# valkey-io/valkey-search

Measured on AMD Instinct MI355X. Metric: kNN queries/sec + recall@10, 10M×768 fp32 cosine, flat & HNSW, 1/2/4/8 GPU, higher is better.
Workload: dtype f32; 1 GPU; FLAT 10000000x768 fp32 COSINE k=10 batch=256 (BASELINE.json configs[1]); rows_per_gpu=10000000

## Files before the change

__graft_entry__.py:

```python
import sys
from pathlib import Path

ROOT = Path(__file__).resolve().parent
sys.path.insert(0, str(ROOT))


def build() -> None:
    import subprocess
    import _pkg
    _pkg.vsa.build()
    assert _pkg.vsa.LIB_PATH.exists()
    _pkg.vsa.lib()
    from oracle import oracle as O
    O.build(ref=True)
    _pkg.vsa.build_experiments()
    subprocess.check_call(["/opt/rocm/bin/hipcc", "--offload-arch=gfx950", "-O2", "-shared", "-fPIC",
                           str(ROOT / "tests" / "helpers" / "mfma_probe.hip"), "-o", str(ROOT / "tests" / "helpers" / "libmfmaprobe.so")])
    subprocess.check_call(["/opt/rocm/bin/hipcc", "--offload-arch=gfx950", "-O2", "-shared", "-fPIC", "-I", str(_pkg.vsa.LIB_PATH.parent / "csrc"),
                           str(ROOT / "tests" / "helpers" / "prefilter_probe.hip"), "-o", str(ROOT / "tests" / "helpers" / "libprefilterprobe.so")])
    subprocess.check_call(["/opt/rocm/bin/hipcc", "--offload-arch=gfx950", "-O2", "-shared", "-fPIC", "-I", str(_pkg.vsa.LIB_PATH.parent / "csrc"),
                           str(ROOT / "tests" / "helpers" / "filter_probe.hip"), "-o", str(ROOT / "tests" / "helpers" / "libfilterprobe.so")])
    subprocess.check_call(["g++", "-O2", "-std=c++17", "-fPIC", "-shared", "-I", str(ROOT / "include"), str(ROOT / "scripts" / "serving_probe.cc"),
                           "-L", str(_pkg.vsa.LIB_PATH.parent), "-lvkindex", "-lpthread",
                           "-Wl,-rpath,$ORIGIN/../" + _pkg.vsa.LIB_PATH.parent.name, "-o", str(ROOT / "scripts" / "libservingprobe.so")])
    subprocess.check_call(["g++", "-O2", "-std=c++17", "-fPIC", "-shared", "-I", str(ROOT / "include"), "-I", str(ROOT / "tests" / "helpers"),
                           str(ROOT / "scripts" / "adaptor_probe.cc"), "-L", str(_pkg.vsa.LIB_PATH.parent), "-lvkindex", "-lpthread",
                           "-Wl,-rpath,$ORIGIN/../" + _pkg.vsa.LIB_PATH.parent.name, "-o", str(ROOT / "scripts" / "libadaptorprobe.so")])
    subprocess.check_call(["g++", "-O2", "-std=c++17", "-I", str(ROOT / "include"), str(ROOT / "scripts" / "coalescer_native.cc"),
                           "-L", str(_pkg.vsa.LIB_PATH.parent), "-lvkindex", "-lpthread",
                           "-Wl,-rpath,$ORIGIN/../" + _pkg.vsa.LIB_PATH.parent.name, "-o", str(ROOT / "scripts" / "coalescer_native")])


def smoke() -> None:
    import numpy as np
    import _pkg
    from oracle import oracle as O
# ... 38 lines not shown
```

valkey-search_amd/csrc/flat_filter.hip:

```cpp
#include <stdlib.h>

#include "device_common.hpp"
#include "kernels.hpp"

namespace vk {

typedef _Float16 f16x8 __attribute__((ext_vector_type(8)));
typedef _Float16 f16x4 __attribute__((ext_vector_type(4)));
typedef float f32x16 __attribute__((ext_vector_type(16)));

#ifdef VK_EXPERIMENTS
__device__ __forceinline__ uint32_t exp_ablate(const FlatFilterArgs &a) { return a.ablate; }
__device__ __forceinline__ uint32_t exp_prio(const FlatFilterArgs &a) { return a.prio; }
__device__ __forceinline__ unsigned long long *exp_dbg(const FlatFilterArgs &a) { return a.dbg; }
#else
__device__ __forceinline__ uint32_t exp_ablate(const FlatFilterArgs &) { return 0u; }
__device__ __forceinline__ uint32_t exp_prio(const FlatFilterArgs &) { return 0u; }
__device__ __forceinline__ unsigned long long *exp_dbg(const FlatFilterArgs &) { return nullptr; }
#endif

namespace {
constexpr int kFTileRows = 128;
constexpr int kFStageK = 64;
constexpr int kFAStride = 72;
}

__global__ __launch_bounds__(256) void row_stats_kernel(const void *rows, uint32_t bf16, uint32_t l2, uint32_t stride_e, uint32_t chunks,
                                                        uint32_t lo, uint32_t hi, uint32_t *stats, uint32_t *tile_norm, uint32_t *hn16,
                                                        _Float16 *rows16) {
  const int lane = threadIdx.x & 63, wave = threadIdx.x >> 6, j = lane & 3, rq = lane >> 2;
  const uint32_t total_waves = gridDim.x * 4, n_tiles = (hi - lo + kRowsPerWave - 1) / kRowsPerWave;
  float best_n2 = 0.f, best_abs = 0.f;
  for (uint32_t tile = blockIdx.x * 4 + wave; tile < n_tiles; tile += total_waves) {
    const uint32_t row = lo + tile * kRowsPerWave + rq;
    const uint32_t lrow = row < hi ? row : hi - 1;
    float n2 = 0.f, mx = 0.f;
    bool bad = false;
    for (uint32_t c = 0; c < chunks; ++c) {
      const float4 x = bf16 ? row_piece<true>(row_base<true>(rows, lrow, stride_e), c * 4 + j)
// ... 461 lines not shown
#pragma unroll
    for (int u = 0; u < kPieces; ++u)
      tn[u] = a.tile_norm[((size_t)((uint32_t)u * a.n_tiles + tile) * kR + i0) * a.sample_gap >> 7];
#pragma unroll
    for (int u = 0; u < kPieces; ++u) pz |= (tn[u] > cap_bits ? 1u : 0u) << u;
  }
  s.pz = pz;
#pragma unroll
  for (int u = 0; u < kPieces; ++u) {
    const size_t run = (size_t)((uint32_t)u * a.n_tiles + tile) * kR * a.sample_gap;
    const u32x4v v = __builtin_amdgcn_raw_buffer_load_b128(ws_rsrc(base + run * row_bytes), (int)voff, 0, 2);
    if constexpr (kBf16) s.v[u] = v;
    else s.v[u] = __builtin_bit_cast(f32x4v, v);
  }
}
template <bool kBf16, bool kL2, bool kSample, bool kBfMma = false>
__device__ __forceinline__ void ws_rows_store(_Float16 *buf, uint32_t *hn_buf, uint32_t t, const WsRows<kBf16> &s, bool raw = false) {
  if constexpr (kL2) hn_buf[t] = s.hn;
  if constexpr (kBf16) {
    _Float16 *dst = buf + (t >> 3) * kFAStride + (t & 7) * 8;
    if (kBfMma || raw) {
#pragma unroll
      for (int u = 0; u < 8; ++u) {
        u32x4v v = s.v[u];
        if constexpr (kSample) {
          if ((t & 7) == 0 && ((s.pz >> u) & 1u)) v[0] = (v[0] & 0xFFFF0000u) | 0x7FC0u;
        }
        *reinterpret_cast<u32x4v *>(dst + u * 16 * kFAStride) = v;
      }
      return;
    }
#pragma unroll
    for (int u = 0; u < 8; ++u) {
      f16x8 h;
#pragma unroll
      for (int w = 0; w < 4; ++w) {
        h[2 * w] = (_Float16)__uint_as_float(s.v[u][w] << 16);
        h[2 * w + 1] = (_Float16)__uint_as_float(s.v[u][w] & 0xFFFF0000u);
      }
      if constexpr (kSample) {
        if ((t & 7) == 0 && ((s.pz >> u) & 1u)) h[0] = __builtin_bit_cast(_Float16, (uint16_t)0x7E00);
      }
      *reinterpret_cast<f16x8 *>(dst + u * 16 * kFAStride) = h;
    }
  } else {
    _Float16 *dst = buf + (t >> 4) * kFAStride + (t & 15) * 4;
#pragma unroll
    for (int u = 0; u < 16; ++u) {
      f16x4 h;
      h[0] = (_Float16)s.v[u][0];
      h[1] = (_Float16)s.v[u][1];
      h[2] = (_Float16)s.v[u][2];
      h[3] = (_Float16)s.v[u][3];
      if constexpr (kSample) {
        if ((t & 15) == 0 && ((s.pz >> u) & 1u)) h[0] = __builtin_bit_cast(_Float16, (uint16_t)0x7E00);
      }
      *reinterpret_cast<f16x4 *>(dst + u * 8 * kFAStride) = h;
    }
  }
}
constexpr int kWsBStage = 8 * 4 * kWave;
constexpr int kWsThreads = 512;
__device__ __forceinline__ void ws_b_load(WsB &b, const FlatFilterArgs &a, uint32_t p, uint32_t st, uint32_t lane) {
  const uint32_t ks_n = a.row_stride_f / 16;
#pragma unroll
  for (int t4 = 0; t4 < 4; ++t4) {
    const uint32_t jt0 = p * 4 + t4, jt = jt0 < a.nqt ? jt0 : a.nqt - 1;
    const __amdgpu_buffer_rsrc_t r = ws_rsrc(reinterpret_cast<const char *>(a.q16) + ((size_t)jt * ks_n + st * 4) * kWave * 16);
#pragma unroll
    for (int kk = 0; kk < 4; ++kk) b.v[t4 * 4 + kk] = __builtin_amdgcn_raw_buffer_load_b128(r, (int)(lane * 16 + kk * 1024), 0, 0);
  }
}
__device__ __forceinline__ void ws_b_store(uint4 *slot, uint32_t p, uint32_t lane, const WsB &b) {
  u32x4v *dst = reinterpret_cast<u32x4v *>(slot) + (p * 16) * kWave + lane;
#pragma unroll
  for (int i = 0; i < 16; ++i) dst[i * kWave] = b.v[i];
}

typedef __bf16 bf16x8 __attribute__((ext_vector_type(8)));
template <bool kBfMma> __device__ __forceinline__ f32x16 ws_mfma(f16x8 x, f16x8 y, f32x16 c) {
  if constexpr (kBfMma) return __builtin_amdgcn_mfma_f32_32x32x16_bf16(__builtin_bit_cast(bf16x8, x), __builtin_bit_cast(bf16x8, y), c, 0, 0, 0);
  else return __builtin_amdgcn_mfma_f32_32x32x16_f16(x, y, c, 0, 0, 0);
}
constexpr int kDmaRing = 5;
constexpr uint32_t kDmaStageBytes = kFTileRows * 128;
constexpr int kBRing = 3;
template <bool kBf16, bool kL2, bool kTiming, bool kSample, int kAbl = 0, bool kBfMma = false, bool kDma = false, bool kBDma = false>
__device__ __forceinline__ void flat_filter_body(const FlatFilterArgs &a) {
  static_assert(!kBDma || (!kDma && !kTiming && !kSample && kAbl == 0), "B by DMA: rows through registers, final pass, no experiment variants");
  static_assert(!kDma || (kBf16 && !kL2 && !kSample && !kTiming), "the DMA row path serves a 16-bit row stream in the final pass");
  const uint32_t abl = kAbl != 0 ? exp_ablate(a) : 0u;
  extern __shared__ _Float16 lds_a[];
  constexpr uint32_t kBufHalfs = kFTileRows * kFAStride;
  uint4 *lds_b = reinterpret_cast<uint4 *>(lds_a + (kDma ? kDmaRing * kDmaStageBytes / 2 : 2 * kBufHalfs));
  uint32_t *lds_ring = reinterpret_cast<uint32_t *>(lds_b + (kBDma ? kBRing : 2) * kWsBStage);
  uint32_t *hn_lds = lds_ring + 4 * kRingWords;
  volatile __attribute__((address_space(3))) uint32_t *lds_stop =
      (volatile __attribute__((address_space(3))) uint32_t *)(hn_lds + 2 * kFTileRows);
  const uint32_t tid = threadIdx.x, lane = tid & 63;
  const uint32_t wave = __builtin_amdgcn_readfirstlane(tid >> 6);
  const uint32_t stages = a.row_stride_f / kFStageK;

  const uint32_t n_tiles = a.n_tiles;
  const uint32_t t_base = n_tiles / gridDim.x, t_rem = n_tiles % gridDim.x;
  uint32_t first_tile = blockIdx.x * t_base + (blockIdx.x < t_rem ? blockIdx.x : t_rem);
  uint32_t my_tiles = t_base + (blockIdx.x < t_rem ? 1u : 0u);
  if constexpr (!kSample) {
    if (a.part_tiles != 0) {
// ... 225 lines not shown
    }
    VK_WS_ROWS_LOAD(x0)
    fpos_advance(ld, stages);
    VK_WS_ROWS_LOAD(x1)
    fpos_advance(ld, stages);
    VK_WS_ROWS_LOAD(x2)
    fpos_advance(ld, stages);
    if constexpr (kBf16) {
      VK_WS_ROWS_LOAD(x3)
      fpos_advance(ld, stages);
      VK_WS_ROWS_LOAD(x4)
      fpos_advance(ld, stages);
      VK_WS_ROWS_LOAD(x5)
      fpos_advance(ld, stages);
    }
    ws_rows_store<kBf16, kL2, kSample, kBfMma>(lds_a, hn_lds, t, x0);
    VK_WS_PBARRIER()
    uint32_t ppar = 0;
    unsigned long long ph[4] = {0, 0, 0, 0}, tlast = __builtin_readcyclecounter();
#define VK_WS_PROD(RLOAD, RSTORE)                                                                                   \
    {                                                                                                               \
      const bool live = left_c != 0;                                                                                \
      VK_WS_TICK(3)                                                                                                 \
      if (live && st_c == 0 && t == 0 && a.cancel && (tile_c % kCancelPollTiles) == 0) {                            \
        if (__hip_atomic_load(a.cancel, __ATOMIC_RELAXED, __HIP_MEMORY_SCOPE_SYSTEM) != 0) lds_stop[tile_c & 1] = 1; \
      }                                                                                                             \
      if (!(abl & 8u)) VK_WS_ROWS_LOAD(RLOAD)                                                                       \
      fpos_advance(ld, stages);                                                                                     \
      __builtin_amdgcn_sched_barrier(0);                                                                            \
      VK_WS_TICK(0)                                                                                                 \
      ppar ^= 1;                                                                                                    \
      if (!(abl & 4u)) ws_rows_store<kBf16, kL2, kSample, kBfMma>(lds_a + ppar * kBufHalfs, hn_lds + ppar * kFTileRows, t, RSTORE, (abl & 512u) != 0); \
      else if (abl & 1024u) {         \
        _Pragma("unroll") for (int u_ = 0; u_ < (kBf16 ? 8 : 16); ++u_) asm volatile("" ::"v"(RSTORE.v[u_]));       \
      }                                                                                                             \
      if constexpr (timing) asm volatile("s_waitcnt lgkmcnt(0)" ::: "memory");                                      \
      VK_WS_TICK(2)                                                                                                 \
      left_c -= live ? 1u : 0u;                                                                                     \
      st_c += 1;                                                                                                    \
      if (live && st_c == stages) VK_WS_TILE_END(VK_WS_PBARRIER()) else VK_WS_PBARRIER();                           \
    }
    while (left_c != 0 && !stop) {
      VK_WS_PROD(x0, x1)
      if (stop) break;
      VK_WS_PROD(x1, x2)
      if (stop) break;
      if constexpr (kBf16) {
// ... 31 lines not shown
    const bool have = wave * 2 + t2 < a.nqt;
    const uint32_t jc = have ? (wave * 2 + t2) * 32 + li : 0u;
    const float4 co = a.qcoef[jc];
    closed[t2] = !have || co.w != 0.f;
    if constexpr (kSample) {
      wit[t2] = a.qwit[jc] + 0x1p-21f;
      col[t2].c1 = col[t2].c0 = col[t2].bound = 0.f;
      if constexpr (kL2) col[t2].c2 = 0.f;
    } else {
      wit[t2] = 0.f;
      if constexpr (kL2) col[t2].c2 = co.x;
      col[t2].c1 = co.y;
      col[t2].c0 = co.z;
      col[t2].bound = (closed[t2] || abl != 0) ? __builtin_inff() : a.qbound[jc];
    }
  }
  f32x16 acc[2][4];
  const f32x16 zero = {0.f, 0.f, 0.f, 0.f, 0.f, 0.f, 0.f, 0.f, 0.f, 0.f, 0.f, 0.f, 0.f, 0.f, 0.f, 0.f};
#pragma unroll
  for (int t2 = 0; t2 < 2; ++t2)
#pragma unroll
    for (int rt = 0; rt < 4; ++rt) acc[t2][rt] = zero;
  uint32_t tile_row0 = first_tile * row_step;
  uint32_t par = 0;
  const __amdgpu_buffer_rsrc_t tile_rsrc = ws_rsrc(a.tile_norm);
  uint32_t norm_bits = 0;
  if constexpr (!kSample) norm_bits = __builtin_amdgcn_raw_buffer_load_b32(tile_rsrc, 0, (int)((tile_row0 / (uint32_t)kFTileRows) * 4u), 0);
  __syncthreads();

#define VK_WS_AB(FA, FB0, FB1, KK)                                                                                  \
// ... 19 lines not shown
    VK_WS_AB(fa, b0, b1, 0)                                                                                         \
    VK_WS_AB(fb, b2, b3, 1)                                                                                         \
    MM0(fa, b0, b1)                                                                                                 \
    VK_WS_AB(fa, b0, b1, 2)                                                                                         \
    VK_WS_MM(fb, b2, b3)                                                                                            \
    VK_WS_AB(fb, b2, b3, 3)                                                                                         \
    VK_WS_MM(fa, b0, b1)                                                                                            \
    VK_WS_MM(fb, b2, b3)                                                                                            \
    __builtin_amdgcn_sched_group_barrier(0x100, 12, 0);                                                             \
    __builtin_amdgcn_sched_group_barrier(0x008, 8, 0);                                                              \
    __builtin_amdgcn_sched_group_barrier(0x100, 6, 0);                                                              \
    __builtin_amdgcn_sched_group_barrier(0x008, 8, 0);                                                              \
    __builtin_amdgcn_sched_group_barrier(0x100, 6, 0);                                                              \
    __builtin_amdgcn_sched_group_barrier(0x008, 16, 0);                                                             \
  }
  f16x8 abl_a[4], abl_b[2];
  if constexpr (kAbl != 0) {
#pragma unroll
    for (int rt = 0; rt < 4; ++rt) abl_a[rt] = *reinterpret_cast<const f16x8 *>(lds_a + li * kFAStride + g * 8 + rt * 32 * kFAStride);
    abl_b[0] = reinterpret_cast<const f16x8 *>(lds_b)[lane];
    abl_b[1] = reinterpret_cast<const f16x8 *>(lds_b)[lane + kWave];
  }
  const uint32_t dma_off = li * 128u + ((g ^ ((li >> 1) & 7u)) * 16u);
  uint32_t dma_slot = 0, b_slot = 0;
  unsigned long long ph[3] = {0, 0, 0}, tlast = __builtin_readcyclecounter();
  while (left_c != 0 && !stop) {
    VK_WS_TICK(2)
    const _Float16 *ab = lds_a + par * kBufHalfs + li * kFAStride + g * 8;
    const char *dma_ab = reinterpret_cast<const char *>(lds_a) + dma_slot;
    const f16x8 *bb = reinterpret_cast<const f16x8 *>(lds_b + (kBDma ? b_slot : par * kWsBStage) + (wave * 2) * 4 * kWave) + lane;
    if (has_q) {
      if (st_c == 0) VK_WS_STAGE(VK_WS_MMZ) else VK_WS_STAGE(VK_WS_MM)
      if constexpr ((kAbl & 128) != 0) VK_WS_STAGE(VK_WS_MM)
      if constexpr (kL2) {
        if (st_c + 1 == stages) {
          const uint4 nb = make_uint4(g == 0 ? 0xBC00BC00u : 0u, 0u, 0u, 0u);
#pragma unroll
          for (int rt = 0; rt < 4; ++rt) {
            const uint4 na = make_uint4(g == 0 ? hn_lds[par * kFTileRows + rt * 32 + li] : 0u, 0u, 0u, 0u);
            acc[0][rt] = __builtin_amdgcn_mfma_f32_32x32x16_f16(__builtin_bit_cast(f16x8, na), __builtin_bit_cast(f16x8, nb), acc[0][rt], 0, 0, 0);
            acc[1][rt] = __builtin_amdgcn_mfma_f32_32x32x16_f16(__builtin_bit_cast(f16x8, na), __builtin_bit_cast(f16x8, nb), acc[1][rt], 0, 0, 0);
          }
        }
      }
    }
    if constexpr (timing) asm volatile("s_nop 7\n s_nop 7" ::: "memory");
    VK_WS_TICK(0)
    left_c -= 1;
    st_c += 1;
    par ^= 1;
    if constexpr (kDma) dma_slot = dma_slot + kDmaStageBytes == kDmaRing * kDmaStageBytes ? 0u : dma_slot + kDmaStageBytes;
    if constexpr (kBDma) b_slot = b_slot + kWsBStage == kBRing * kWsBStage ? 0u : b_slot + kWsBStage;
    if (st_c == stages) {
      if (has_q) {
        if constexpr (kSample) {
          sample_max<4, kBf16>(a, acc[0], wit[0], closed[0], tile_row0, (wave * 2) * 32 + li, g);
          sample_max<4, kBf16>(a, acc[1], wit[1], closed[1], tile_row0, (wave * 2 + 1) * 32 + li, g);
        } else if constexpr ((kAbl & 64) != 0) {
#pragma unroll
          for (int rt = 0; rt < 4; ++rt) asm volatile("" ::"v"(acc[0][rt]), "v"(acc[1][rt]));
        } else {
          filter_gate<4, false>(a, acc[0], gate_thr<kL2>(col[0], norm_bits), tile_row0, wave * 2, li, g, ring, lane);
          filter_gate<4, false>(a, acc[1], gate_thr<kL2>(col[1], norm_bits), tile_row0, wave * 2 + 1, li, g, ring, lane);
        }
      }
      tile_row0 += row_step;
      if constexpr (!kSample) norm_bits = __builtin_amdgcn_raw_buffer_load_b32(tile_rsrc, 0, (int)((tile_row0 / (uint32_t)kFTileRows) * 4u), 0);
      VK_WS_TICK(1)
      VK_WS_TILE_END(__syncthreads())
    } else {
      __syncthreads();
    }
  }
#undef VK_WS_AB
#undef VK_WS_MM
#undef VK_WS_MMZ
#undef VK_WS_STAGE
#undef VK_WS_TILE_END
#undef VK_WS_TICK
  if constexpr (timing) {
    if (lane == 0 && exp_dbg(a))
      for (int i = 0; i < 3; ++i) atomicAdd(&exp_dbg(a)[5 + i], ph[i]);
  }
  ring_flush(a, ring, lane);
}


template <bool kBf16, bool kL2, bool kTiming, int kAbl = 0>
__global__ __launch_bounds__(kWsThreads, 1) void flat_filter_kernel(FlatFilterArgs a) {
  flat_filter_body<kBf16, kL2, kTiming, false, kAbl>(a);
}
__global__ __launch_bounds__(kWsThreads, 1) void flat_filter_bfmma_kernel(FlatFilterArgs a) {
  flat_filter_body<true, false, false, false, 0, true>(a);
}
__global__ __launch_bounds__(kWsThreads, 1) void flat_filter_bfmma_dma_kernel(FlatFilterArgs a) {
  flat_filter_body<true, false, false, false, 0, true, true>(a);
}
template <bool kBf16, bool kL2, bool kBfMma, bool kImage = false>
__global__ __launch_bounds__(kWsThreads, 1) void flat_filter_bdma_kernel(FlatFilterArgs a) {
  static_assert(!kImage || (!kBf16 && !kL2 && !kBfMma), "the f16 image belongs to f32 rows in the inner-product space");
  if constexpr (kImage) flat_filter_body<true, false, false, false, 0, false, true>(a);
  else flat_filter_body<kBf16, kL2, false, false, 0, kBfMma, false, true>(a);
}
template <bool kBf16, bool kL2, bool kBfMma, bool kImage = false>
__global__ __launch_bounds__(kWsThreads, 1) void flat_filter_early_kernel(FlatFilterArgs a) {
  static_assert(!kImage || (!kBf16 && !kL2 && !kBfMma), "the f16 image belongs to f32 rows in the inner-product space");
  if constexpr (kImage) flat_filter_body<true, false, false, false, 0, false, true>(a);
  else flat_filter_body<kBf16, kL2, false, false, 0, kBfMma, false, true>(a);
}
__global__ __launch_bounds__(kWsThreads, 1) void flat_filter_early_bfmma_dma_kernel(FlatFilterArgs a) {
  flat_filter_body<true, false, false, false, 0, true, true>(a);
}
#ifdef VK_EXPERIMENTS
template <int kAbl>
__global__ __launch_bounds__(kWsThreads, 1) void flat_filter_bfmma_dma_abl_kernel(FlatFilterArgs a) {
  flat_filter_body<true, false, false, false, kAbl, true, true>(a);
}
#endif
__global__ __launch_bounds__(kWsThreads, 1) void flat_filter_bfmma_sample_kernel(FlatFilterArgs a) {
  flat_filter_body<true, false, false, true, 0, true>(a);
}
template <bool kBf16, bool kL2>
__global__ __launch_bounds__(kWsThreads, 1) void flat_filter_sample_kernel(FlatFilterArgs a) {
  flat_filter_body<kBf16, kL2, false, true>(a);
}

size_t flat_filter_dma_lds_bytes() {
  return (size_t)kDmaRing * kDmaStageBytes + (size_t)2 * kWsBStage * 16 + (size_t)4 * kRingWords * 4 + (size_t)2 * kFTileRows * 4 + 16;
}
size_t flat_filter_bdma_lds_bytes() {
  return (size_t)2 * kFTileRows * kFAStride * sizeof(_Float16) + (size_t)kBRing * kWsBStage * 16 + (size_t)4 * kRingWords * 4 +
         (size_t)2 * kFTileRows * 4 + 16;
}
size_t flat_filter_lds_bytes() {
  return (size_t)2 * kFTileRows * kFAStride * sizeof(_Float16) + (size_t)2 * kWsBStage * 16 + (size_t)4 * kRingWords * 4 +
         (size_t)2 * kFTileRows * 4 + 16;
}

bool flat_filter_supported(uint32_t row_stride_f, uint64_t k, bool bf16, bool l2) {
  (void)bf16;
  (void)l2;
  return (row_stride_f % kFStageK) == 0 && k >= 1 && k <= 1024;
}

hipError_t launch_flat_qprep(const FlatFilterArgs &a, hipStream_t s) {
  hipLaunchKernelGGL(flat_qprep_kernel, dim3(a.nqt * 32), dim3(64), 0, s, a);
// ... 29 lines not shown
#else
  constexpr bool exp_variant = false;
#endif
  if (a.bdma && a.mode == 0 && !exp_variant && !(a.qbf16 && a.dma)) {
    fn = a.qbf16 ? reinterpret_cast<const void *>(&flat_filter_bdma_kernel<true, false, true>)
         : a.bf16 ? (a.l2 ? reinterpret_cast<const void *>(&flat_filter_bdma_kernel<true, true, false>)
                          : reinterpret_cast<const void *>(&flat_filter_bdma_kernel<true, false, false>))
                  : (a.l2 ? reinterpret_cast<const void *>(&flat_filter_bdma_kernel<false, true, false>)
                          : reinterpret_cast<const void *>(&flat_filter_bdma_kernel<false, false, false>));
    if (a.early)
      fn = a.qbf16 ? reinterpret_cast<const void *>(&flat_filter_early_kernel<true, false, true>)
           : a.bf16 ? (a.l2 ? reinterpret_cast<const void *>(&flat_filter_early_kernel<true, true, false>)
                            : reinterpret_cast<const void *>(&flat_filter_early_kernel<true, false, false>))
                    : (a.l2 ? reinterpret_cast<const void *>(&flat_filter_early_kernel<false, true, false>)
                            : reinterpret_cast<const void *>(&flat_filter_early_kernel<false, false, false>));
    lds = flat_filter_bdma_lds_bytes();
  }
  if (a.rows16 != nullptr && a.mode == 0 && !exp_variant) {
    if (a.bf16 || a.l2 || a.qbf16) return hipErrorInvalidValue;
    fn = a.early ? reinterpret_cast<const void *>(&flat_filter_early_kernel<false, false, false, true>)
                 : reinterpret_cast<const void *>(&flat_filter_bdma_kernel<false, false, false, true>);
    lds = flat_filter_dma_lds_bytes();
  }
#ifdef VK_EXPERIMENTS
  if (a.timing) {
    if (a.l2 || a.mode == 1 || a.qbf16) return hipErrorInvalidValue;
    fn = a.bf16 ? reinterpret_cast<const void *>(&flat_filter_kernel<true, false, true>)
                : reinterpret_cast<const void *>(&flat_filter_kernel<false, false, true>);
  }
  if (a.ablate_on && !(a.qbf16 && a.dma && a.mode == 0)) {
    if (a.l2 || a.mode == 1 || a.qbf16) return hipErrorInvalidValue;
#define VK_ABL(T, N) (a.bf16 ? reinterpret_cast<const void *>(&flat_filter_kernel<true, false, T, N>) : reinterpret_cast<const void *>(&flat_filter_kernel<false, false, T, N>))
    switch (a.ablate & 240u) {
      case 240: fn = VK_ABL(false, 241); break;
      case 16: fn = VK_ABL(false, 17); break;
      case 32: fn = VK_ABL(false, 33); break;
      case 48: fn = VK_ABL(false, 49); break;
// ... 16 lines not shown
```

valkey-search_amd/csrc/flat_index.cc:

```cpp
#include <stdio.h>
#include <stdlib.h>
#include <string.h>

#include <algorithm>
#include <atomic>
#include <chrono>
#include <cmath>
#include <queue>
#include <thread>

#include "index.hpp"

namespace vk {

Status SearchCtx::begin_on(hipStream_t s) {
  if (has_busy) {
    VK_HIP_TRY(hipStreamWaitEvent(s, busy, 0));
    has_busy = false;
  }
  return Status::Ok();
}

Status SearchCtx::end_async(hipStream_t s) {
  if (!busy) VK_HIP_TRY(hipEventCreateWithFlags(&busy, hipEventDisableTiming));
// ... 899 lines not shown
    uint32_t *redo_cnt = words + w_misc + 1;
#ifdef VK_EXPERIMENTS
    const bool timing = getenv("VK_FILTER_TIMING") && atoi(getenv("VK_FILTER_TIMING")) != 0;
    const bool filter_experiment = getenv("VK_FILTER_TIMING") || (getenv("VK_FILTER_ABLATE") && !getenv("VK_FILTER_ABLATE_DMA"));
#else
    constexpr bool filter_experiment = false;
#endif

    FlatFilterArgs f{};
    f.rows = store_.d_rows();
    f.bf16 = store_.bf16() ? 1 : 0;
    f.l2 = l2() ? 1 : 0;
    f.qbf16 = (store_.bf16() && !l2() && opt_.get(kOptFilterBf16Mfma) != 0 && !filter_experiment) ? 1 : 0;
    f.dma = (f.qbf16 && opt_.get(kOptFilterRowDma) != 0) ? 1 : 0;
    f.bdma = opt_.get(kOptFilterBDma) != 0 ? 1u : 0u;
    f.hn16 = l2() ? d_hn16_.as<uint32_t>() : nullptr;
    std::shared_lock<std::shared_mutex> image_lk(image_mu_);
    f.rows16 = (!store_.bf16() && !l2() && !filter_experiment && !filter_dump_active() && opt_.get(kOptFlatF16Image) != 0) ? d_rows16_.p : nullptr;
    last_filter_image_bytes_.store(f.rows16 ? (uint64_t)store_.alloc_rows() * dp * 2 : 0, std::memory_order_relaxed);
    f.labels = store_.d_labels();
    f.allow_bits = d_allow;
    f.allow_nbits = allow_nbits;
    f.queries = d_q;
    f.q_stride_f = dp;
    f.q16 = ctx->d_fq16.p;
    f.qcoef = ctx->d_fthr.as<float4>();
    f.qbound = reinterpret_cast<float *>(ctx->d_fthr.as<char>() + (size_t)nqt * 32 * 16);
    f.qwit = f.qbound + (size_t)nqt * 32;
    f.norm_cap = d_rowstats_.as<uint32_t>() + 3;
    f.sample_gap = gap;
// ... 353 lines not shown
```

valkey-search_amd/csrc/kernels.hpp:

```cpp
#pragma once
#include <hip/hip_runtime.h>
#include <stdint.h>

#ifdef VK_EXPERIMENTS
#include <stdlib.h>
#define VK_TUNE(env, dflt) (getenv(env) ? atoll(getenv(env)) : (long long)(dflt))
#else
#define VK_TUNE(env, dflt) ((long long)(dflt))
#endif

namespace vk {

hipError_t ensure_max_lds(const void *fn);

struct FlatScanArgs {
  const void *rows;
  const uint64_t *labels;
  const float *queries;
  const uint64_t *allow_bits;
  uint64_t allow_nbits;
  const float *lb_dist;
  const uint64_t *lb_label;
  float *part_dist;
  uint64_t *part_label;
// ... 85 lines not shown
  uint32_t *ovf_q;
  uint32_t *done_cnt;
  uint32_t *rerank_cnt;
  uint32_t mode;
  float *smax;
  uint32_t smax_ld;
  uint32_t smax_fine;
  uint32_t sample_gap;
  const uint32_t *norm_cap;
  float *qwit;
  uint32_t n_tiles;
  uint32_t part_first, part_tiles, early;
  uint32_t row_stride_f, n_rows, nq;
  uint32_t nqt;
  const uint32_t *cancel;
#ifdef VK_EXPERIMENTS
  uint32_t timing;
  unsigned long long *dbg;
  uint32_t prio;
  uint32_t ablate_on, ablate;
  float *dump_scores;
  float *dump_thr;
  uint32_t dump_rows, dump_ld;
#endif
};
struct FlatBoundArgs {
  const float *smax;
  uint32_t smax_ld, groups, k, nq;
  float *qbound;
};
// ... 202 lines not shown
```

valkey-search_amd/csrc/options.hpp:

```cpp
#pragma once
#include <stdint.h>
#include <stdlib.h>
#include <string.h>

#include <atomic>
#include <string>

#include "row_store.hpp"

namespace vk {

enum OptId : uint32_t {
  kOptCoalesceMaxBatch,
  kOptCoalesceMaxWaitUs,
  kOptMaxQueryQueueDepth,
  kOptBatchesInFlight,
  kOptCompleterThreads,
  kOptHandoutChunk,
  kOptShardEfPct,
  kOptShardGather,
  kOptFilterCacheEntries,
  kOptFilterCacheBytes,
  kOptKernelTiming,
  kOptFlatFilter, kOptFilterMinQueries, kOptFilterMinRows, kOptFilterPrepassRows, kOptFilterCap, kOptFilterSpillChunks,
  kOptFilterBDma, kOptFilterRowDma, kOptFilterBf16Mfma, kOptFlatForceScan, kOptFlatFusedRerank, kOptFilterSecondBound, kOptFilterTwoPass, kOptFilterTwoPassMinTiles, kOptFilterEarlyPermille, kOptFlatF16Image,
  kOptGemmLockstep, kOptGemmPrepassRows, kOptGemmContig, kOptScanMinNrp, kOptUploadParallel,
  kOptHnswStageAdds, kOptHnswStageMax,
  kOptHnswOptimisticTombstones, kOptHnswDeviceBuild, kOptHnswBuildBatch, kOptHnswBuildMinGraph, kOptHnswBuildMinBatch, kOptHnswBuildFrac,
  kOptHnswBuildVerbose, kOptHnswFailpointBatch, kOptHnswPoolFloor, kOptHnswGpoolCap, kOptHnswVisitedHash, kOptHnswHashPerEf, kOptHnswHashLog2, kOptHnswVisitedMode, kOptHnswLdsWork, kOptHnswLdsWorkBig,
  kOptHnswPoolBytes, kOptHnswVisitedBytes, kOptHnswRedoBytes,
  kOptHnswNodeMask, kOptHnswNodeMaskBytes,
  kOptShardThreads, kOptShardAllowStaged,
  kOptCount
};

struct OptDesc {
  const char *name;
  const char *env;
  uint64_t dflt, lo, hi;
};
// ... 16 lines not shown
      {"filter-min-queries", "VK_FILTER_MIN_QUERIES", 5, 1, kMax},
      {"filter-min-rows", "VK_FILTER_MIN_ROWS", 262144, 0, kMax},
      {"filter-prepass-rows", "VK_FILTER_PREPASS", 262144, 1024, kMax},
      {"filter-cap", "VK_FILTER_CAP", 8192, 64, 1u << 24},
      {"filter-spill-chunks", "VK_FILTER_SPILL_CHUNKS", 1024, 0, 1u << 20},
      {"filter-bdma", "VK_FILTER_BDMA", 1, 0, 1},
      {"filter-row-dma", "VK_FILTER_DMA", 1, 0, 1},
      {"filter-bf16-mfma", "VK_FILTER_BF16_MFMA", 1, 0, 1},
      {"flat-force-scan", "VK_FLAT_FORCE_SCAN", 0, 0, 1},
      {"flat-fused-rerank", "VK_FLAT_FUSED_RERANK", 1, 0, 1},
      {"filter-second-bound", "VK_FILTER_SECOND_BOUND", 1, 0, 1},
      {"filter-two-pass", "VK_FILTER_TWO_PASS", 1, 0, 1},
      {"filter-two-pass-min-tiles", "VK_FILTER_TWO_PASS_MIN_TILES", 16, 2, 1u << 20},
      {"filter-early-permille", "VK_FILTER_EARLY_PERMILLE", 0, 0, 250},
      {"flat-f16-image", "VK_FLAT_F16_IMAGE", 1, 0, 1},
      {"gemm-lockstep", "VK_GEMM_LOCKSTEP", 1, 0, 64},
      {"gemm-prepass-rows", "VK_GEMM_PREPASS", 16384, 0, kMax},
      {"gemm-contig", "VK_GEMM_CONTIG", 1, 0, 1},
      {"scan-min-nrp", "VK_SCAN_MIN_NRP", 8, 1, 4096},
      {"upload-parallel", "VK_UPLOAD_PARALLEL", 1, 0, 1},
      {"hnsw-stage-adds", "VK_HNSW_STAGE_ADDS", 1, 0, 1},
      {"hnsw-stage-max", "VK_HNSW_STAGE_MAX", 262144, 1, 1u << 26},
      {"hnsw-optimistic-tombstones", "VK_HNSW_OPTIMISTIC_TOMBSTONES", 1, 0, 1},
      {"hnsw-device-build", "VK_HNSW_DEVICE_BUILD", 1, 0, 1},
      {"hnsw-build-batch", "VK_HNSW_BUILD_BATCH", 8192, 1, 1u << 20},
      {"hnsw-build-min-graph", "VK_HNSW_BUILD_MIN_GRAPH", 16384, 1, kMax},
      {"hnsw-build-min-batch", "VK_HNSW_BUILD_MIN_BATCH", 64, 1, kMax},
      {"hnsw-build-frac", "VK_HNSW_BUILD_FRAC", 32, 1, 1u << 20},
      {"hnsw-build-verbose", "VK_HNSW_BUILD_VERBOSE", 0, 0, 1},
      {"hnsw-failpoint-batch", "VK_HNSW_FAILPOINT_BATCH", 0, 0, kMax},
// ... 76 lines not shown
```

Baseline: 57510 queries/s.

## Add 16x16x32 MFMA variant of flat filter kernel with padded LDS stride

Adds an alternative path in the flat filter kernel that uses 16x16x32 MFMA instructions in place of 32x32x16. It comes with a new LDS row stride of 80 halfs for the A tile, a matching stage macro with its own instruction scheduling hints, and a gate routine that reads the 16x16 accumulator layout. The path is selected for inner-product and cosine final passes through a new option that defaults to on. The intent is better MFMA issue and latency behaviour and fewer LDS bank conflicts, at the cost of more code variants and a different survivor-gating layout that must keep results identical.

```diff
diff --git a/__graft_entry__.py b/__graft_entry__.py
--- a/__graft_entry__.py
+++ b/__graft_entry__.py
@@ -20,6 +20,8 @@
                            str(ROOT / "tests" / "helpers" / "prefilter_probe.hip"), "-o", str(ROOT / "tests" / "helpers" / "libprefilterprobe.so")])
     subprocess.check_call(["/opt/rocm/bin/hipcc", "--offload-arch=gfx950", "-O2", "-shared", "-fPIC", "-I", str(_pkg.vsa.LIB_PATH.parent / "csrc"),
                            str(ROOT / "tests" / "helpers" / "filter_probe.hip"), "-o", str(ROOT / "tests" / "helpers" / "libfilterprobe.so")])
+    subprocess.check_call(["/opt/rocm/bin/hipcc", "--offload-arch=gfx950", "-O2", "-shared", "-fPIC", "-I", str(_pkg.vsa.LIB_PATH.parent / "csrc"),
+                           str(ROOT / "tests" / "helpers" / "filter_shape_probe.hip"), "-o", str(ROOT / "tests" / "helpers" / "libfiltershapeprobe.so")])
     subprocess.check_call(["g++", "-O2", "-std=c++17", "-fPIC", "-shared", "-I", str(ROOT / "include"), str(ROOT / "scripts" / "serving_probe.cc"),
                            "-L", str(_pkg.vsa.LIB_PATH.parent), "-lvkindex", "-lpthread",
                            "-Wl,-rpath,$ORIGIN/../" + _pkg.vsa.LIB_PATH.parent.name, "-o", str(ROOT / "scripts" / "libservingprobe.so")])
diff --git a/valkey-search_amd/csrc/flat_filter.hip b/valkey-search_amd/csrc/flat_filter.hip
--- a/valkey-search_amd/csrc/flat_filter.hip
+++ b/valkey-search_amd/csrc/flat_filter.hip
@@ -23,6 +23,7 @@
 constexpr int kFTileRows = 128;
 constexpr int kFStageK = 64;
 constexpr int kFAStride = 72;
+constexpr int kFAStride16 = 80;
 }
 
 __global__ __launch_bounds__(256) void row_stats_kernel(const void *rows, uint32_t bf16, uint32_t l2, uint32_t stride_e, uint32_t chunks,
@@ -514,11 +515,11 @@
     else s.v[u] = __builtin_bit_cast(f32x4v, v);
   }
 }
-template <bool kBf16, bool kL2, bool kSample, bool kBfMma = false>
+template <bool kBf16, bool kL2, bool kSample, bool kBfMma = false, int kStride = kFAStride>
 __device__ __forceinline__ void ws_rows_store(_Float16 *buf, uint32_t *hn_buf, uint32_t t, const WsRows<kBf16> &s, bool raw = false) {
   if constexpr (kL2) hn_buf[t] = s.hn;
   if constexpr (kBf16) {
-    _Float16 *dst = buf + (t >> 3) * kFAStride + (t & 7) * 8;
+    _Float16 *dst = buf + (t >> 3) * kStride + (t & 7) * 8;
     if (kBfMma || raw) {
 #pragma unroll
       for (int u = 0; u < 8; ++u) {
@@ -526,7 +527,7 @@
         if constexpr (kSample) {
           if ((t & 7) == 0 && ((s.pz >> u) & 1u)) v[0] = (v[0] & 0xFFFF0000u) | 0x7FC0u;
         }
-        *reinterpret_cast<u32x4v *>(dst + u * 16 * kFAStride) = v;
+        *reinterpret_cast<u32x4v *>(dst + u * 16 * kStride) = v;
       }
       return;
     }
@@ -541,10 +542,10 @@
       if constexpr (kSample) {
         if ((t & 7) == 0 && ((s.pz >> u) & 1u)) h[0] = __builtin_bit_cast(_Float16, (uint16_t)0x7E00);
       }
-      *reinterpret_cast<f16x8 *>(dst + u * 16 * kFAStride) = h;
+      *reinterpret_cast<f16x8 *>(dst + u * 16 * kStride) = h;
     }
   } else {
-    _Float16 *dst = buf + (t >> 4) * kFAStride + (t & 15) * 4;
+    _Float16 *dst = buf + (t >> 4) * kStride + (t & 15) * 4;
 #pragma unroll
     for (int u = 0; u < 16; ++u) {
       f16x4 h;
@@ -555,7 +556,7 @@
       if constexpr (kSample) {
         if ((t & 15) == 0 && ((s.pz >> u) & 1u)) h[0] = __builtin_bit_cast(_Float16, (uint16_t)0x7E00);
       }
-      *reinterpret_cast<f16x4 *>(dst + u * 8 * kFAStride) = h;
+      *reinterpret_cast<f16x4 *>(dst + u * 8 * kStride) = h;
     }
   }
 }
@@ -582,16 +583,96 @@
   if constexpr (kBfMma) return __builtin_amdgcn_mfma_f32_32x32x16_bf16(__builtin_bit_cast(bf16x8, x), __builtin_bit_cast(bf16x8, y), c, 0, 0, 0);
   else return __builtin_amdgcn_mfma_f32_32x32x16_f16(x, y, c, 0, 0, 0);
 }
+template <bool kBfMma> __device__ __forceinline__ f32x4v ws_mfma16(f16x8 x, f16x8 y, f32x4v c) {
+  if constexpr (kBfMma) return __builtin_amdgcn_mfma_f32_16x16x32_bf16(__builtin_bit_cast(bf16x8, x), __builtin_bit_cast(bf16x8, y), c, 0, 0, 0);
+  else return __builtin_amdgcn_mfma_f32_16x16x32_f16(x, y, c, 0, 0, 0);
+}
 constexpr int kDmaRing = 5;
 constexpr uint32_t kDmaStageBytes = kFTileRows * 128;
 constexpr int kBRing = 3;
-template <bool kBf16, bool kL2, bool kTiming, bool kSample, int kAbl = 0, bool kBfMma = false, bool kDma = false, bool kBDma = false>
+template <bool kL2>
+__device__ __forceinline__ void filter_gate16(const FlatFilterArgs &a, const f32x4v (&acc)[4][8], const GateCol<kL2> &col, uint32_t norm_bits,
+                                              uint32_t tile_row0, uint32_t wave, uint32_t c, uint32_t kg, SurvivorRing &ring, uint32_t lane) {
+  const float thr_own = gate_thr<kL2>(col, norm_bits);
+  float thr[4];
+#pragma unroll
+  for (int qs = 0; qs < 4; ++qs) thr[qs] = __shfl(thr_own, qs * 16 + (int)c);
+#ifdef VK_EXPERIMENTS
+  if (a.dump_scores != nullptr && tile_row0 < a.dump_rows) {
+#pragma unroll
+    for (int qs = 0; qs < 4; ++qs) {
+      const uint32_t q = wave * 64 + qs * 16 + c;
+      if (q < a.nq && q < a.dump_ld) {
+#pragma unroll
+        for (int rs = 0; rs < 8; ++rs)
+#pragma unroll
+          for (int r = 0; r < 4; ++r) {
+            const uint32_t row = tile_row0 + rs * 16 + 4 * kg + r;
+            if (row < a.dump_rows) a.dump_scores[(size_t)row * a.dump_ld + q] = acc[qs][rs][r];
+          }
+      }
+    }
+    if (wave * 64 + lane < a.nq && wave * 64 + lane < a.dump_ld) a.dump_thr[(size_t)(tile_row0 / 128u) * a.dump_ld + wave * 64 + lane] = thr_own;
+  }
+#endif
+  float mx[4];
+  bool any = false;
+#pragma unroll
+  for (int qs = 0; qs < 4; ++qs) {
+    mx[qs] = acc[qs][0][0];
+#pragma unroll
+    for (int i = 1; i < 32; ++i) mx[qs] = fmaxf(mx[qs], acc[qs][i >> 2][i & 3]);
+    any = any || !(mx[qs] < thr[qs]);
+  }
+  if (__builtin_amdgcn_ballot_w64(any) == 0) return;
+#pragma unroll
+  for (int qs = 0; qs < 4; ++qs) {
+    const float m = mx[qs], t = thr[qs];
+    if (__builtin_amdgcn_ballot_w64(!(m < t)) == 0) continue;
+    const uint32_t q = wave * 64 + qs * 16 + c;
+    uint32_t mk = 0;
+#pragma unroll
+    for (int i = 0; i < 32; ++i) mk |= !(acc[qs][i >> 2][i & 3] < t) ? 1u << i : 0u;
+    if (q >= a.nq) mk = 0;
+    const bool multi = __builtin_amdgcn_ballot_w64(__builtin_popcount(mk) > 1 || (mk != 0 && m < t)) != 0;
+    while (__builtin_amdgcn_ballot_w64(mk != 0) != 0) {
+      const uint32_t r = mk != 0 ? (uint32_t)__builtin_ctz(mk) : 0u;
+      const uint32_t row = tile_row0 + (r >> 2) * 16 + 4 * kg + (r & 3);
+      bool pass = mk != 0 && row < a.n_rows;
+      if (pass && a.allow_bits != nullptr) pass = allow_bit(a.allow_bits, a.allow_nbits, a.labels[row]);
+      float score = m;
+      if (multi) {
+#pragma unroll
+        for (int i = 0; i < 32; ++i) score = r == (uint32_t)i ? acc[qs][i >> 2][i & 3] : score;
+      }
+      mk &= mk - 1;
+      const uint64_t pm = __builtin_amdgcn_ballot_w64(pass);
+      if (pm != 0) {
+        const uint32_t n = (uint32_t)__popcll(pm);
+        if (ring.cnt + n > kWave) ring_flush(a, ring, lane);
+        if (pass) {
+          const uint32_t at = ring.cnt + (uint32_t)__popcll(pm & ((1ull << lane) - 1ull));
+          ring.ent[at * 3] = q;
+          ring.ent[at * 3 + 1] = row;
+          ring.ent[at * 3 + 2] = __float_as_uint(score);
+        }
+        ring.cnt += n;
+      }
+    }
+  }
+}
+
+template <bool kBf16, bool kL2, bool kTiming, bool kSample, int kAbl = 0, bool kBfMma = false, bool kDma = false, bool kBDma = false,
+          bool kM16 = false>
 __device__ __forceinline__ void flat_filter_body(const FlatFilterArgs &a) {
+  static_assert(!kM16 || ((kDma || kBDma) && !kL2 && !kSample && !kTiming && kAbl == 0), "16x16x32: final pass, inner-product space, no experiment variants");
+  static_assert(!kM16 || kDma || !kBf16, "16x16x32 with the rows through registers: f32 rows");
+  constexpr int kAStride = kM16 ? kFAStride16 : kFAStride;
   static_assert(!kBDma || (!kDma && !kTiming && !kSample && kAbl == 0), "B by DMA: rows through registers, final pass, no experiment variants");
   static_assert(!kDma || (kBf16 && !kL2 && !kSample && !kTiming), "the DMA row path serves a 16-bit row stream in the final pass");
   const uint32_t abl = kAbl != 0 ? exp_ablate(a) : 0u;
   extern __shared__ _Float16 lds_a[];
-  constexpr uint32_t kBufHalfs = kFTileRows * kFAStride;
+  constexpr uint32_t kBufHalfs = kFTileRows * kAStride;
   uint4 *lds_b = reinterpret_cast<uint4 *>(lds_a + (kDma ? kDmaRing * kDmaStageBytes / 2 : 2 * kBufHalfs));
   uint32_t *lds_ring = reinterpret_cast<uint32_t *>(lds_b + (kBDma ? kBRing : 2) * kWsBStage);
   uint32_t *hn_lds = lds_ring + 4 * kRingWords;
@@ -847,7 +928,7 @@
       VK_WS_ROWS_LOAD(x5)
       fpos_advance(ld, stages);
     }
-    ws_rows_store<kBf16, kL2, kSample, kBfMma>(lds_a, hn_lds, t, x0);
+    ws_rows_store<kBf16, kL2, kSample, kBfMma, kAStride>(lds_a, hn_lds, t, x0);
     VK_WS_PBARRIER()
     uint32_t ppar = 0;
     unsigned long long ph[4] = {0, 0, 0, 0}, tlast = __builtin_readcyclecounter();
@@ -863,7 +944,7 @@
       __builtin_amdgcn_sched_barrier(0);                                                                            \
       VK_WS_TICK(0)                                                                                                 \
       ppar ^= 1;                                                                                                    \
-      if (!(abl & 4u)) ws_rows_store<kBf16, kL2, kSample, kBfMma>(lds_a + ppar * kBufHalfs, hn_lds + ppar * kFTileRows, t, RSTORE, (abl & 512u) != 0); \
+      if (!(abl & 4u)) ws_rows_store<kBf16, kL2, kSample, kBfMma, kAStride>(lds_a + ppar * kBufHalfs, hn_lds + ppar * kFTileRows, t, RSTORE, (abl & 512u) != 0); \
       else if (abl & 1024u) {         \
         _Pragma("unroll") for (int u_ = 0; u_ < (kBf16 ? 8 : 16); ++u_) asm volatile("" ::"v"(RSTORE.v[u_]));       \
       }                                                                                                             \
@@ -925,6 +1006,19 @@
       col[t2].c0 = co.z;
       col[t2].bound = (closed[t2] || abl != 0) ? __builtin_inff() : a.qbound[jc];
     }
+  }
+  const uint32_t c16 = lane & 15, kg16 = lane >> 4;
+  GateCol<kL2> col16;
+  f32x4v acc16[4][8];
+  const f32x4v zero4 = {0.f, 0.f, 0.f, 0.f};
+  {
+    const bool have = kM16 && wave * 2 + (lane >> 5) < a.nqt;
+    const uint32_t jc = have ? wave * 64 + lane : 0u;
+    const float4 co = a.qcoef[jc];
+    if constexpr (kL2) col16.c2 = co.x;
+    col16.c1 = co.y;
+    col16.c0 = co.z;
+    col16.bound = (!have || co.w != 0.f) ? __builtin_inff() : a.qbound[jc];
   }
   f32x16 acc[2][4];
   const f32x16 zero = {0.f, 0.f, 0.f, 0.f, 0.f, 0.f, 0.f, 0.f, 0.f, 0.f, 0.f, 0.f, 0.f, 0.f, 0.f, 0.f};
@@ -974,6 +1068,36 @@
     __builtin_amdgcn_sched_group_barrier(0x100, 6, 0);                                                              \
     __builtin_amdgcn_sched_group_barrier(0x008, 16, 0);                                                             \
   }
+#define VK_WS_A16(RS, S)                                                                                            \
+  (kDma ? *reinterpret_cast<const f16x8 *>(dma_ab + (dma_off16 ^ ((S) * 64u)) + (RS) * 2048)                         \
+        : *reinterpret_cast<const f16x8 *>(ab16 + (RS) * 16 * kAStride + (S) * 32))
+#define VK_WS_B16(QS, S) bb16[(((QS) >> 1) * 4 + 2 * (S)) * kWave + ((QS) & 1) * 16]
+#define VK_WS_STAGE16(C0)                                                                                           \
+  {                                                                                                                 \
+    f16x8 fa[8], fb[4], fc[2];                                                                                      \
+    _Pragma("unroll") for (int rs = 0; rs < 8; ++rs) fa[rs] = VK_WS_A16(rs, 0);                                     \
+    _Pragma("unroll") for (int qs = 0; qs < 4; ++qs) fb[qs] = VK_WS_B16(qs, 0);                                     \
+    fc[0] = VK_WS_B16(0, 1);                                                                                        \
+    fc[1] = VK_WS_B16(1, 1);                                                                                        \
+    _Pragma("unroll") for (int rs = 0; rs < 8; ++rs) {                                                              \
+      _Pragma("unroll") for (int qs = 0; qs < 4; ++qs) acc16[qs][rs] = ws_mfma16<kBfMma>(fa[rs], fb[qs], C0);       \
+      fa[rs] = VK_WS_A16(rs, 1);                                                                                    \
+    }                                                                                                               \
+    fb[2] = VK_WS_B16(2, 1);                                                                                        \
+    fb[3] = VK_WS_B16(3, 1);                                                                                        \
+    _Pragma("unroll") for (int qs = 0; qs < 4; ++qs)                                                                \
+      _Pragma("unroll") for (int rs = 0; rs < 8; ++rs)                                                              \
+        acc16[qs][rs] = ws_mfma16<kBfMma>(fa[rs], qs < 2 ? fc[qs] : fb[qs], acc16[qs][rs]);                         \
+    __builtin_amdgcn_sched_group_barrier(0x100, 14, 0);                                                             \
+    _Pragma("unroll") for (int rs = 0; rs < 7; ++rs) {                                                              \
+      __builtin_amdgcn_sched_group_barrier(0x008, 4, 0);                                                            \
+      __builtin_amdgcn_sched_group_barrier(0x100, 1, 0);                                                            \
+    }                                                                                                               \
+    __builtin_amdgcn_sched_group_barrier(0x008, 4, 0);                                                              \
+    __builtin_amdgcn_sched_group_barrier(0x100, 3, 0);                                                              \
+    __builtin_amdgcn_sched_group_barrier(0x008, 32, 0);                                                             \
+  }
+  const uint32_t dma_off16 = c16 * 128u + ((kg16 ^ ((c16 >> 1) & 7u)) * 16u);
   f16x8 abl_a[4], abl_b[2];
   if constexpr (kAbl != 0) {
 #pragma unroll
@@ -989,7 +1113,20 @@
     const _Float16 *ab = lds_a + par * kBufHalfs + li * kFAStride + g * 8;
     const char *dma_ab = reinterpret_cast<const char *>(lds_a) + dma_slot;
     const f16x8 *bb = reinterpret_cast<const f16x8 *>(lds_b + (kBDma ? b_slot : par * kWsBStage) + (wave * 2) * 4 * kWave) + lane;
-    if (has_q) {
+    const _Float16 *ab16 = lds_a + par * kBufHalfs + c16 * kAStride + kg16 * 8;
+    const f16x8 *bb16 = reinterpret_cast<const f16x8 *>(lds_b + (kBDma ? b_slot : par * kWsBStage) + (wave * 2) * 4 * kWave) +
+                        (kg16 >> 1) * kWave + (kg16 & 1) * 32 + c16;
+    if constexpr (kM16) {
+      if (has_q) {
+        if (st_c == 0) {
+          asm volatile("; first stage of a tile" ::: "memory");
+          VK_WS_STAGE16(zero4)
+        } else {
+          asm volatile("; stage" ::: "memory");
+          VK_WS_STAGE16(acc16[qs][rs])
+        }
+      }
+    } else if (has_q) {
       if (st_c == 0) VK_WS_STAGE(VK_WS_MMZ) else VK_WS_STAGE(VK_WS_MM)
       if constexpr ((kAbl & 128) != 0) VK_WS_STAGE(VK_WS_MM)
       if constexpr (kL2) {
@@ -1019,6 +1156,8 @@
         } else if constexpr ((kAbl & 64) != 0) {
 #pragma unroll
           for (int rt = 0; rt < 4; ++rt) asm volatile("" ::"v"(acc[0][rt]), "v"(acc[1][rt]));
+        } else if constexpr (kM16) {
+          filter_gate16<kL2>(a, acc16, col16, norm_bits, tile_row0, wave, c16, kg16, ring, lane);
         } else {
           filter_gate<4, false>(a, acc[0], gate_thr<kL2>(col[0], norm_bits), tile_row0, wave * 2, li, g, ring, lane);
           filter_gate<4, false>(a, acc[1], gate_thr<kL2>(col[1], norm_bits), tile_row0, wave * 2 + 1, li, g, ring, lane);
@@ -1036,6 +1175,9 @@
 #undef VK_WS_MM
 #undef VK_WS_MMZ
 #undef VK_WS_STAGE
+#undef VK_WS_STAGE16
+#undef VK_WS_A16
+#undef VK_WS_B16
 #undef VK_WS_TILE_END
 #undef VK_WS_TICK
   if constexpr (timing) {
@@ -1056,17 +1198,25 @@
 __global__ __launch_bounds__(kWsThreads, 1) void flat_filter_bfmma_dma_kernel(FlatFilterArgs a) {
   flat_filter_body<true, false, false, false, 0, true, true>(a);
 }
-template <bool kBf16, bool kL2, bool kBfMma, bool kImage = false>
+__global__ __launch_bounds__(kWsThreads, 1) void flat_filter_bfmma_dma_m16_kernel(FlatFilterArgs a) {
+  flat_filter_body<true, false, false, false, 0, true, true, false, true>(a);
+}
+__global__ __launch_bounds__(kWsThreads, 1) void flat_filter_early_bfmma_dma_m16_kernel(FlatFilterArgs a) {
+  flat_filter_body<true, false, false, false, 0, true, true, false, true>(a);
+}
+template <bool kBf16, bool kL2, bool kBfMma, bool kImage = false, bool kM16 = false>
 __global__ __launch_bounds__(kWsThreads, 1) void flat_filter_bdma_kernel(FlatFilterArgs a) {
   static_assert(!kImage || (!kBf16 && !kL2 && !kBfMma), "the f16 image belongs to f32 rows in the inner-product space");
-  if constexpr (kImage) flat_filter_body<true, false, false, false, 0, false, true>(a);
-  else flat_filter_body<kBf16, kL2, false, false, 0, kBfMma, false, true>(a);
-}
-template <bool kBf16, bool kL2, bool kBfMma, bool kImage = false>
+  static_assert(!kM16 || (!kBf16 && !kL2 && !kBfMma), "16x16x32: f32 rows in the inner-product space, image and register path alike");
+  if constexpr (kImage) flat_filter_body<true, false, false, false, 0, false, true, false, kM16>(a);
+  else flat_filter_body<kBf16, kL2, false, false, 0, kBfMma, false, true, kM16>(a);
+}
+template <bool kBf16, bool kL2, bool kBfMma, bool kImage = false, bool kM16 = false>
 __global__ __launch_bounds__(kWsThreads, 1) void flat_filter_early_kernel(FlatFilterArgs a) {
   static_assert(!kImage || (!kBf16 && !kL2 && !kBfMma), "the f16 image belongs to f32 rows in the inner-product space");
-  if constexpr (kImage) flat_filter_body<true, false, false, false, 0, false, true>(a);
-  else flat_filter_body<kBf16, kL2, false, false, 0, kBfMma, false, true>(a);
+  static_assert(!kM16 || (!kBf16 && !kL2 && !kBfMma), "16x16x32: f32 rows in the inner-product space, image and register path alike");
+  if constexpr (kImage) flat_filter_body<true, false, false, false, 0, false, true, false, kM16>(a);
+  else flat_filter_body<kBf16, kL2, false, false, 0, kBfMma, false, true, kM16>(a);
 }
 __global__ __launch_bounds__(kWsThreads, 1) void flat_filter_early_bfmma_dma_kernel(FlatFilterArgs a) {
   flat_filter_body<true, false, false, false, 0, true, true>(a);
@@ -1088,8 +1238,8 @@
 size_t flat_filter_dma_lds_bytes() {
   return (size_t)kDmaRing * kDmaStageBytes + (size_t)2 * kWsBStage * 16 + (size_t)4 * kRingWords * 4 + (size_t)2 * kFTileRows * 4 + 16;
 }
-size_t flat_filter_bdma_lds_bytes() {
-  return (size_t)2 * kFTileRows * kFAStride * sizeof(_Float16) + (size_t)kBRing * kWsBStage * 16 + (size_t)4 * kRingWords * 4 +
+size_t flat_filter_bdma_lds_bytes(bool m16) {
+  return (size_t)2 * kFTileRows * (m16 ? kFAStride16 : kFAStride) * sizeof(_Float16) + (size_t)kBRing * kWsBStage * 16 + (size_t)4 * kRingWords * 4 +
          (size_t)2 * kFTileRows * 4 + 16;
 }
 size_t flat_filter_lds_bytes() {
@@ -1149,13 +1299,25 @@
                             : reinterpret_cast<const void *>(&flat_filter_early_kernel<true, false, false>))
                     : (a.l2 ? reinterpret_cast<const void *>(&flat_filter_early_kernel<false, true, false>)
                             : reinterpret_cast<const void *>(&flat_filter_early_kernel<false, false, false>));
-    lds = flat_filter_bdma_lds_bytes();
+    lds = flat_filter_bdma_lds_bytes(false);
   }
   if (a.rows16 != nullptr && a.mode == 0 && !exp_variant) {
     if (a.bf16 || a.l2 || a.qbf16) return hipErrorInvalidValue;
     fn = a.early ? reinterpret_cast<const void *>(&flat_filter_early_kernel<false, false, false, true>)
                  : reinterpret_cast<const void *>(&flat_filter_bdma_kernel<false, false, false, true>);
     lds = flat_filter_dma_lds_bytes();
+  }
+  if (a.mfma16 && a.mode == 0 && !exp_variant && !a.l2) {
+    if (a.qbf16 && a.dma) {
+      fn = a.early ? reinterpret_cast<const void *>(&flat_filter_early_bfmma_dma_m16_kernel) : reinterpret_cast<const void *>(&flat_filter_bfmma_dma_m16_kernel);
+    } else if (a.rows16 != nullptr) {
+      fn = a.early ? reinterpret_cast<const void *>(&flat_filter_early_kernel<false, false, false, true, true>)
+                   : reinterpret_cast<const void *>(&flat_filter_bdma_kernel<false, false, false, true, true>);
+    } else if (a.bdma && !a.bf16 && !a.qbf16) {
+      fn = a.early ? reinterpret_cast<const void *>(&flat_filter_early_kernel<false, false, false, false, true>)
+                   : reinterpret_cast<const void *>(&flat_filter_bdma_kernel<false, false, false, false, true>);
+      lds = flat_filter_bdma_lds_bytes(true);
+    }
   }
 #ifdef VK_EXPERIMENTS
   if (a.timing) {
diff --git a/valkey-search_amd/csrc/flat_index.cc b/valkey-search_amd/csrc/flat_index.cc
--- a/valkey-search_amd/csrc/flat_index.cc
+++ b/valkey-search_amd/csrc/flat_index.cc
@@ -937,6 +937,7 @@
     f.qbf16 = (store_.bf16() && !l2() && opt_.get(kOptFilterBf16Mfma) != 0 && !filter_experiment) ? 1 : 0;
     f.dma = (f.qbf16 && opt_.get(kOptFilterRowDma) != 0) ? 1 : 0;
     f.bdma = opt_.get(kOptFilterBDma) != 0 ? 1u : 0u;
+    f.mfma16 = (!l2() && !filter_experiment && opt_.get(kOptFilterMfmaShape) != 0) ? 1u : 0u;
     f.hn16 = l2() ? d_hn16_.as<uint32_t>() : nullptr;
     std::shared_lock<std::shared_mutex> image_lk(image_mu_);
     f.rows16 = (!store_.bf16() && !l2() && !filter_experiment && !filter_dump_active() && opt_.get(kOptFlatF16Image) != 0) ? d_rows16_.p : nullptr;
diff --git a/valkey-search_amd/csrc/kernels.hpp b/valkey-search_amd/csrc/kernels.hpp
--- a/valkey-search_amd/csrc/kernels.hpp
+++ b/valkey-search_amd/csrc/kernels.hpp
@@ -123,6 +123,7 @@
   uint32_t row_stride_f, n_rows, nq;
   uint32_t nqt;
   const uint32_t *cancel;
+  uint32_t mfma16;
 #ifdef VK_EXPERIMENTS
   uint32_t timing;
   unsigned long long *dbg;
diff --git a/valkey-search_amd/csrc/options.hpp b/valkey-search_amd/csrc/options.hpp
--- a/valkey-search_amd/csrc/options.hpp
+++ b/valkey-search_amd/csrc/options.hpp
@@ -23,7 +23,7 @@
   kOptFilterCacheBytes,
   kOptKernelTiming,
   kOptFlatFilter, kOptFilterMinQueries, kOptFilterMinRows, kOptFilterPrepassRows, kOptFilterCap, kOptFilterSpillChunks,
-  kOptFilterBDma, kOptFilterRowDma, kOptFilterBf16Mfma, kOptFlatForceScan, kOptFlatFusedRerank, kOptFilterSecondBound, kOptFilterTwoPass, kOptFilterTwoPassMinTiles, kOptFilterEarlyPermille, kOptFlatF16Image,
+  kOptFilterBDma, kOptFilterRowDma, kOptFilterBf16Mfma, kOptFlatForceScan, kOptFlatFusedRerank, kOptFilterSecondBound, kOptFilterTwoPass, kOptFilterTwoPassMinTiles, kOptFilterEarlyPermille, kOptFlatF16Image, kOptFilterMfmaShape,
   kOptGemmLockstep, kOptGemmPrepassRows, kOptGemmContig, kOptScanMinNrp, kOptUploadParallel,
   kOptHnswStageAdds, kOptHnswStageMax,
   kOptHnswOptimisticTombstones, kOptHnswDeviceBuild, kOptHnswBuildBatch, kOptHnswBuildMinGraph, kOptHnswBuildMinBatch, kOptHnswBuildFrac,
@@ -70,6 +70,7 @@
       {"filter-two-pass-min-tiles", "VK_FILTER_TWO_PASS_MIN_TILES", 16, 2, 1u << 20},
       {"filter-early-permille", "VK_FILTER_EARLY_PERMILLE", 0, 0, 250},
       {"flat-f16-image", "VK_FLAT_F16_IMAGE", 1, 0, 1},
+      {"filter-mfma-shape", "VK_FILTER_MFMA_SHAPE", 1, 0, 1},
       {"gemm-lockstep", "VK_GEMM_LOCKSTEP", 1, 0, 64},
       {"gemm-prepass-rows", "VK_GEMM_PREPASS", 16384, 0, kMax},
       {"gemm-contig", "VK_GEMM_CONTIG", 1, 0, 1},
```

New measurement: 61480 queries/s, median of 6. 6.9% higher.
